# jluuser/PyTorch-VAE

Hardware: AMD Instinct MI355X
Metric: train images/sec @64x64x3 bs256 (curve tensors [B,64,6], SURVEY.md s0) (higher is better)
Workload: dtype f32; 1 GPU; C2: stage2_vq.yaml model with num_quantizers=1 K=512 D=64 N=64; full train step (fwd+loss+bwd+clip+AdamW+EMA), dropout 0.1, loss weights at epoch 100; per_gpu_batch=256, global_batch=256, seq_len=64, parallelism=dp1, hipgraph=True, params=43115078

## Files before the change

pytorch-vae_amd/csrc/loss.hip:

```cpp
#include "common.h"

namespace {

enum { T_VALID = 0, T_PAIR = 1, T_TRI = 2, T_QUAD = 3, T_FIVE = 4, T_ANY3 = 5, T_PDM = 8, T_LR = 40 };

enum {
    P_RAW = 0, P_ALN, P_BEST, P_RMSD_RAW, P_RMSD_BEST, P_CE, P_ACC, P_SSTV, P_BL, P_BA, P_DIR, P_DIH, P_TV2, P_TAU,
    P_PDM, P_LRPDM, P_WINK, P_COMMIT, P_KAPPA, P_COUNT
};

enum {
    M_LOSS = 0, M_REC_XYZ, M_MSE_RAW, M_MSE_ALN, M_REC_SS, M_SS_ACC, M_VQ_LOSS, M_BL, M_BA, M_DIR, M_DIH, M_GEOM,
    M_SS_TV, M_USAGE_REG, M_TV2, M_PPL, M_DEAD, M_RMSD_RAW, M_RMSD_ALN, M_PDM, M_WINK, M_KAPPA, M_TAU, M_LRPDM, M_COUNT
};

struct LossCfg {
    int B, L, Ntok, D;
    int Ls;
    const float* Ldev;
    int masked;
    int use_vq;
    float rmsd_w, ss_w, bl_w, ba_w, dir_w, dih_w, tv_l, pdm_w, wk_w, kap_w, tau_w, lr_w;
    float alpha, ss_tv_l, label_smoothing, beta;
    int pdm_window, wk_size, wk_stride, lr_sep, lr_stride, lr_max;
// ... 187 lines not shown
    }
    sm = block_sum_d(sm, dred);
    const double den = fmax(sm, 1.0);
    double amu[3], bmu[3];
    for (int c = 0; c < 3; ++c) { amu[c] = block_sum_d(sa[c], dred) / den; bmu[c] = block_sum_d(sb[c], dred) / den; }
    double Hm[9] = {0, 0, 0, 0, 0, 0, 0, 0, 0};
    for (int l = threadIdx.x; l < n; l += blockDim.x) {
        const double w = m[l0 + l];
        double ac[3], bc[3];
        for (int c = 0; c < 3; ++c) {
            ac[c] = (double)((float)a[3 * (l0 + l) + c] - (float)amu[c]);
            bc[c] = (double)((float)b[3 * (l0 + l) + c] - (float)bmu[c]);
        }
        for (int i = 0; i < 3; ++i)
            for (int j = 0; j < 3; ++j) Hm[3 * i + j] += w * ac[i] * bc[j];
    }
    for (int k = 0; k < 9; ++k) Hm[k] = block_sum_d(Hm[k], dred);
    if (threadIdx.x == 0) {
        double R[9];
        kabsch_rotation(Hm, R);
        bool ok = true;
        for (int k = 0; k < 9; ++k) { Rt_s[k] = (float)R[k]; ok = ok && isfinite(R[k]); }
        for (int j = 0; j < 3; ++j) {
            const double t = bmu[j] - (amu[0] * R[0 * 3 + j] + amu[1] * R[1 * 3 + j] + amu[2] * R[2 * 3 + j]);
            Rt_s[9 + j] = (float)t;
            ok = ok && isfinite(t);
        }
        Rt_s[12] = ok ? 1.f : 0.f;
    }
    __syncthreads();
    return Rt_s[12] != 0.f;
}

__global__ __launch_bounds__(256) void loss_counts_kernel(const unsigned char* __restrict__ mask, LossCfg c_in,
                                                          int* __restrict__ table) {
    const LossCfg c = loss_resolve(c_in);
    extern __shared__ unsigned char sm_[];
    unsigned char* m = sm_;
    const int b = blockIdx.x, L = c.L;
    for (int l = threadIdx.x; l < L; l += 256) m[l] = mask ? mask[(size_t)b * c.Ls + l] : 1;
    __syncthreads();
    int nv = 0, np = 0, nt = 0, nq = 0, n5 = 0;
    for (int l = threadIdx.x; l < L; l += 256) {
        nv += m[l];
        if (l + 1 < L) np += m[l] & m[l + 1];
        if (l + 2 < L) nt += m[l] & m[l + 1] & m[l + 2];
        if (l + 3 < L) nq += m[l] & m[l + 1] & m[l + 2] & m[l + 3];
        if (l + 4 < L) n5 += m[l] & m[l + 1] & m[l + 2] & m[l + 3] & m[l + 4];
    }
    __shared__ int red[5];
    if (threadIdx.x < 5) red[threadIdx.x] = 0;
    __syncthreads();
    atomicAdd(&red[0], nv); atomicAdd(&red[1], np); atomicAdd(&red[2], nt); atomicAdd(&red[3], nq); atomicAdd(&red[4], n5);
    __syncthreads();
    if (threadIdx.x == 0) {
        atomicAdd(&table[T_VALID], red[0]); atomicAdd(&table[T_PAIR], red[1]); atomicAdd(&table[T_TRI], red[2]);
        atomicAdd(&table[T_QUAD], red[3]); atomicAdd(&table[T_FIVE], red[4]);
        if (red[0] >= 3) atomicAdd(&table[T_ANY3], 1);
    }
    for (int d = 1 + (threadIdx.x >> 6); d < c.pdm_window && d < 32; d += 4) {
        int s = 0;
        for (int l = threadIdx.x & 63; l + d < L; l += 64) s += m[l] & m[l + d];
        for (int o = 32; o > 0; o >>= 1) s += __shfl_xor(s, o, 64);
        if ((threadIdx.x & 63) == 0 && s) atomicAdd(&table[T_PDM + d - 1], s);
    }
    {
        int p = 0;
        for (int off = 0; off < max(1, c.lr_max); ++off)
            for (int i = 0; i < L; i += max(1, c.lr_stride)) {
                const int j = i + c.lr_sep + off;
                if (j >= L) break;
                if ((p & 255) == (int)threadIdx.x && (m[i] & m[j])) atomicAdd(&table[T_LR + p], 1);
                ++p;
            }
    }
    for (int w = threadIdx.x; w < c.n_windows; w += 256) {
        const int s0 = w * max(1, c.wk_stride);
        int cnt = 0;
        for (int l = 0; l < c.wk_size; ++l) cnt += m[s0 + l];
        if (!c.masked || cnt >= 3) atomicAdd(&table[c.t_wk + w], 1);
    }
}

#define FOR_POS(n_) for (int base_ = 0; base_ < (n_); base_ += 256)

__global__ __launch_bounds__(256) void loss_sample_kernel(const float* __restrict__ recons,
                                                          const float* __restrict__ target,
                                                          const unsigned char* __restrict__ mask,
                                                          const float* __restrict__ ze, const float* __restrict__ zq,
                                                          const int* __restrict__ table, LossCfg c_in,
                                                          float* __restrict__ d_recons, float* __restrict__ d_ze,
                                                          float* __restrict__ part) {
    extern __shared__ __attribute__((aligned(16))) float sm[];
    const LossCfg c = loss_resolve(c_in);
    const int L = c.L, b = blockIdx.x, tid = threadIdx.x;
    double* dred = reinterpret_cast<double*>(sm);
    float* rx = sm + 8;
    float* gx = rx + 3 * L;
    float* lg = gx + 3 * L;
    float* pr = lg + 3 * L;
    float* g = pr + 3 * L;
    float* mk = g + 3 * L;
    float* dcs = mk + L;
    float* dhr = dcs + 2 * L;
    float* dhg = dhr + 2 * L;
    int* lab = reinterpret_cast<int*>(dhg + 2 * L);
    float* red = reinterpret_cast<float*>(lab + L);
    float* Rt = red + 4;
    float* rrb = Rt + 16;
    float* grb = rrb + 3 * L;
    float* gRb = grb + 3 * L;
    const float* rr = c.has_stats ? rrb : rx;
    const float* gr = c.has_stats ? grb : gx;
// ... 342 lines not shown
            }
        }
    }
    __syncthreads();

    float commit = 0.f;
    if (c.use_vq && ze) {
        const int n = c.Ntok * c.D;
        const float wq = 2.f * c.beta / ((float)c.B * (float)n);
        const float* zeb = ze + (size_t)b * n;
        const float* zqb = zq + (size_t)b * n;
        float* dzb = d_ze + (size_t)b * n;
        for (int i = tid; i < n; i += 256) {
            const float d = zeb[i] - zqb[i];
            commit += d * d;
            dzb[i] = wq * d;
        }
        commit = block_sum(commit, red);
    }

    float* dxb = d_recons + (size_t)b * c.Ls * 6;
    for (int l = tid; l < L; l += 256)
        for (int k = 0; k < 3; ++k) dxb[6 * l + k] = c.has_stats ? g[3 * l + k] + gRb[3 * l + k] * c.sd[k] : g[3 * l + k];
    for (int i = 6 * L + tid; i < 6 * c.Ls; i += 256) dxb[i] = 0.f;
    if (tid == 0) {
        float* p = part + (size_t)b * P_COUNT;
        p[P_RAW] = raw; p[P_ALN] = aln; p[P_BEST] = best;
        p[P_RMSD_RAW] = sqrtf(fmaxf(raw, 1e-12f)); p[P_RMSD_BEST] = sqrtf(fmaxf(best, 1e-12f));
        p[P_CE] = ce; p[P_ACC] = acc; p[P_SSTV] = sstv; p[P_BL] = bl; p[P_BA] = ba; p[P_DIR] = dr; p[P_DIH] = dih;
        p[P_TV2] = tv2; p[P_TAU] = tau; p[P_KAPPA] = kap; p[P_PDM] = pdm; p[P_LRPDM] = lrp; p[P_WINK] = wink; p[P_COMMIT] = commit;
    }
}

__global__ void loss_finish_kernel(const float* __restrict__ part, const int* __restrict__ table, LossCfg c_in,
                                   const float* __restrict__ vq_stats, float* __restrict__ metrics) {
    const LossCfg c = loss_resolve(c_in);
    __shared__ double acc[P_COUNT];
    if (threadIdx.x < P_COUNT) {
        double s = 0.0;
        for (int b = 0; b < c.B; ++b) s += (double)part[(size_t)b * P_COUNT + threadIdx.x];
        acc[threadIdx.x] = s;
    }
    __syncthreads();
    if (threadIdx.x != 0) return;
    auto cnt = [&](int slot) { return fmax((double)table[slot], 1.0); };
    const double B = c.B;
    const double l_raw = acc[P_RAW] / B, l_aln = acc[P_BEST] / B;
    const double l_xyz = c.alpha * l_aln + (1.0 - c.alpha) * l_raw;
    const double l_ss = acc[P_CE] / cnt(T_VALID);
    const double ss_tv = (c.ss_tv_l > 0.f && c.L >= 2) ? acc[P_SSTV] / cnt(T_PAIR) : 0.0;
    const double bl = c.L >= 2 ? acc[P_BL] / cnt(T_PAIR) : 0.0;
    const double ba = c.L >= 3 ? acc[P_BA] / cnt(T_TRI) : 0.0;
    const double dr = c.L >= 2 ? acc[P_DIR] / cnt(T_PAIR) : 0.0;
    double dih = 0.0;
    if (c.L >= 4) dih = c.masked ? acc[P_DIH] / cnt(T_QUAD) : acc[P_DIH] / (2.0 * B * (c.L - 3));
    const double geom = c.bl_w * bl + c.ba_w * ba + c.dir_w * dr + c.dih_w * dih;
    const double xyz_tv = (c.tv_l > 0.f && c.L >= 3) ? acc[P_TV2] / cnt(T_TRI) : 0.0;
    const double kappa = (c.kap_w > 0.f && c.L >= 3) ? acc[P_KAPPA] / cnt(T_TRI) : 0.0;
    const double tau = (c.tau_w > 0.f && c.L >= 5) ? acc[P_TAU] / cnt(T_FIVE) : 0.0;
    const double vq = c.use_vq ? c.beta * acc[P_COMMIT] / (B * c.Ntok * c.D) : 0.0;
    const double pdm = acc[P_PDM], lrp = acc[P_LRPDM], wink = acc[P_WINK];
    const double total = c.rmsd_w * l_xyz + c.ss_w * l_ss + vq + geom + c.ss_tv_l * ss_tv + c.tv_l * xyz_tv + c.pdm_w * pdm +
                         c.wk_w * wink + c.kap_w * kappa + c.tau_w * tau + c.lr_w * lrp;
    metrics[M_LOSS] = (float)total;
    metrics[M_REC_XYZ] = (float)l_xyz;
    metrics[M_MSE_RAW] = (float)l_raw;
    metrics[M_MSE_ALN] = (float)(acc[P_ALN] / B);
    metrics[M_REC_SS] = (float)l_ss;
    metrics[M_SS_ACC] = (float)(acc[P_ACC] / cnt(T_VALID));
    metrics[M_VQ_LOSS] = (float)vq;
    metrics[M_BL] = (float)bl; metrics[M_BA] = (float)ba; metrics[M_DIR] = (float)dr; metrics[M_DIH] = (float)dih;
    metrics[M_GEOM] = (float)geom;
    metrics[M_SS_TV] = (float)ss_tv;
    metrics[M_USAGE_REG] = 0.f;
    metrics[M_TV2] = (float)xyz_tv;
// ... 9 lines not shown

extern "C" int vqh_loss_fwd_bwd(const float* recons, const float* target, const unsigned char* mask, int masked,
                                const float* ze, const float* zq, const float* vq_stats, int B, int L, int L_stride, const float* L_dev,
                                int Ntok, int D, int use_vq, const float* weights, const int* iparams, const float* data_stats,
                                float* d_recons, float* d_ze, float* metrics, float* workspace,
                                long long workspace_floats, hipStream_t stream) {
    VQH_CHECK_ARG(B > 0 && L > 0 && L_stride >= L, "vqh_loss_fwd_bwd: bad shape");
    VQH_CHECK_ARG(recons && target && weights && iparams && d_recons && metrics && workspace, "vqh_loss_fwd_bwd: null pointer");
    VQH_CHECK_ARG(!use_vq || (ze && zq && d_ze), "vqh_loss_fwd_bwd: VQ tensors missing");
    LossCfg c{};
    c.B = B; c.L = L_dev ? L_stride : L; c.Ls = L_stride; c.Ldev = L_dev; c.Ntok = Ntok; c.D = D; c.masked = masked ? 1 : 0; c.use_vq = use_vq ? 1 : 0;
    c.rmsd_w = weights[0]; c.ss_w = weights[1]; c.bl_w = weights[2]; c.ba_w = weights[3]; c.dir_w = weights[4];
    c.dih_w = weights[5]; c.tv_l = weights[6]; c.pdm_w = weights[7]; c.wk_w = weights[8]; c.kap_w = weights[9];
    c.tau_w = weights[10]; c.lr_w = weights[11]; c.alpha = weights[12]; c.ss_tv_l = weights[13];
    c.label_smoothing = weights[14]; c.beta = weights[15];
    c.pdm_window = iparams[0]; c.wk_size = iparams[1]; c.wk_stride = iparams[2]; c.lr_sep = iparams[3];
    c.lr_stride = iparams[4]; c.lr_max = iparams[5];
    c.has_stats = data_stats ? 1 : 0;
    for (int k = 0; k < 3; ++k) { c.sd[k] = data_stats ? data_stats[k] : 1.f; c.mu[k] = data_stats ? data_stats[3 + k] : 0.f; }
    VQH_CHECK_ARG(c.pdm_window <= 33, "vqh_loss_fwd_bwd: pdm_window > 33 unsupported");
    int npairs = 0, nwin = 0;
    loss_enumerate(L_dev ? L_stride : L, c.lr_sep, c.lr_stride, c.lr_max, c.wk_size, c.wk_stride, &npairs, &nwin);
    c.n_lr_pairs = npairs;
    c.n_windows = nwin;
    c.t_wk = T_LR + npairs;
    const long long table_ints = c.t_wk + nwin + 8;
    const long long need = table_ints + (long long)B * P_COUNT;
    VQH_CHECK_ARG(need <= workspace_floats, "vqh_loss_fwd_bwd: workspace too small");
    int* table = reinterpret_cast<int*>(workspace);
    float* part = workspace + table_ints;
    hipError_t e = hipMemsetAsync(table, 0, sizeof(int) * table_ints, stream);
    if (e != hipSuccess) { vqh_set_error(hipGetErrorString(e)); return VQH_ERR_LAUNCH; }
    const int Lmax = c.L;
    hipLaunchKernelGGL(loss_counts_kernel, dim3(B), dim3(256), (size_t)Lmax, stream, mask, c, table);
    const size_t smem = sizeof(float) * (size_t)(8 + 23 * Lmax + 4 + 16 + 9 * Lmax + 4);
    VQH_CHECK_ARG(smem <= 160 * 1024, "vqh_loss_fwd_bwd: sequence too long for the LDS-resident loss kernel");
    static bool attr_set = false;
    if (!attr_set) {
        hipError_t ea = hipFuncSetAttribute(reinterpret_cast<const void*>(&loss_sample_kernel),
                                            hipFuncAttributeMaxDynamicSharedMemorySize, 160 * 1024);
        if (ea != hipSuccess) { vqh_set_error(hipGetErrorString(ea)); return VQH_ERR_LAUNCH; }
        attr_set = true;
    }
    hipLaunchKernelGGL(loss_sample_kernel, dim3(B), dim3(256), smem, stream, recons, target, mask, ze, zq, table, c,
                       d_recons, d_ze, part);
    hipLaunchKernelGGL(loss_finish_kernel, dim3(1), dim3(64), 0, stream, part, table, c, vq_stats, metrics);
    VQH_LAUNCH_CHECK();
    return VQH_OK;
}
```

pytorch-vae_amd/csrc/rowwise.hip:

```cpp
#include "common.h"
#include <stdlib.h>

namespace {

constexpr int WAVES_PER_BLOCK = 4;

__global__ __launch_bounds__(256) void layernorm_fwd_kernel(const float* __restrict__ x, int ldx,
                                                            const float* __restrict__ w, const float* __restrict__ b,
                                                            float* __restrict__ y, int ldy, float* __restrict__ mean,
                                                            float* __restrict__ rstd, int rows, int H, float eps) {
    const int lane = threadIdx.x & 63;
    const int row = blockIdx.x * WAVES_PER_BLOCK + (threadIdx.x >> 6);
    if (row >= rows) return;
    const float* xr = x + (size_t)row * ldx;
    float s = 0.f;
    for (int i = lane; i < H; i += 64) s += xr[i];
    const float mu = wave_sum(s) / (float)H;
    float v = 0.f;
    for (int i = lane; i < H; i += 64) {
        const float d = xr[i] - mu;
        v += d * d;
    }
    const float rs = rsqrtf(wave_sum(v) / (float)H + eps);
    float* yr = y + (size_t)row * ldy;
    for (int i = lane; i < H; i += 64) yr[i] = (xr[i] - mu) * rs * w[i] + b[i];
    if (lane == 0) {
        if (mean) mean[row] = mu;
        if (rstd) rstd[row] = rs;
    }
}

template <int NV>
__global__ __launch_bounds__(256) void layernorm_fwd_vec_kernel(const float* __restrict__ x, int ldx,
                                                                const float* __restrict__ w, const float* __restrict__ b,
                                                                float* __restrict__ y, int ldy, float* __restrict__ mean,
                                                                float* __restrict__ rstd, int rows, int H, float eps) {
    const int lane = threadIdx.x & 63, wave = threadIdx.x >> 6;
    const int nq = H >> 2;
// ... 209 lines not shown
        for (int j = 0; j < 16; ++j) t += red[j][tx];
        float* o = (i < H) ? dw + i : db + (i - H);
        *o = (beta != 0.f) ? beta * (*o) + t : t;
    }
}

__global__ __launch_bounds__(1024) void reduce_slabs_kernel(const float* __restrict__ slabs, int S, long long stride,
                                                            long long n, float* __restrict__ out, float beta) {
    __shared__ float red[16][64];
    const int tx = threadIdx.x & 63, ty = threadIdx.x >> 6;
    const long long i = (long long)blockIdx.x * 64 + tx;
    float s = 0.f;
    if (i < n) {
        int k = ty;
        for (; k + 48 < S; k += 64) {
            const float a = slabs[(size_t)k * stride + i], b = slabs[(size_t)(k + 16) * stride + i];
            const float c = slabs[(size_t)(k + 32) * stride + i], d = slabs[(size_t)(k + 48) * stride + i];
            s += (a + b) + (c + d);
        }
        for (; k < S; k += 16) s += slabs[(size_t)k * stride + i];
    }
    red[ty][tx] = s;
    __syncthreads();
    if (ty == 0 && i < n) {
        float t = 0.f;
#pragma unroll
        for (int j = 0; j < 16; ++j) t += red[j][tx];
        out[i] = (beta != 0.f) ? beta * out[i] + t : t;
    }
}

__global__ __launch_bounds__(256) void colsum_vec_kernel(const float* __restrict__ X, int ld, int M, int N,
                                                         float* __restrict__ part, int rows_per_block) {
    __shared__ f32x4 red[4][64];
    const int lane = threadIdx.x & 63, ry = threadIdx.x >> 6;
    const int c = blockIdx.x * 256 + lane * 4;
    const int r0 = blockIdx.y * rows_per_block;
    const int r1 = min(M, r0 + rows_per_block);
    f32x4 s0 = {0.f, 0.f, 0.f, 0.f}, s1 = s0;
    if (c < N) {
        int r = r0 + ry;
        for (; r + 4 < r1; r += 8) {
            s0 += *reinterpret_cast<const f32x4*>(X + (size_t)r * ld + c);
            s1 += *reinterpret_cast<const f32x4*>(X + (size_t)(r + 4) * ld + c);
        }
        for (; r < r1; r += 4) s0 += *reinterpret_cast<const f32x4*>(X + (size_t)r * ld + c);
    }
    red[ry][lane] = s0 + s1;
    __syncthreads();
    if (ry == 0 && c < N) {
        const f32x4 t = (red[0][lane] + red[1][lane]) + (red[2][lane] + red[3][lane]);
        *reinterpret_cast<f32x4*>(part + (size_t)blockIdx.y * N + c) = t;
    }
}

__global__ __launch_bounds__(256) void colsum_kernel(const float* __restrict__ X, int ld, int M, int N,
                                                     float* __restrict__ part, int rows_per_block) {
    __shared__ float red[4][64];
    const int c = blockIdx.x * 64 + (threadIdx.x & 63);
    const int ry = threadIdx.x >> 6;
    const int r0 = blockIdx.y * rows_per_block;
    const int r1 = min(M, r0 + rows_per_block);
    float s = 0.f;
    if (c < N)
        for (int r = r0 + ry; r < r1; r += 4) s += X[(size_t)r * ld + c];
    red[ry][threadIdx.x & 63] = s;
    __syncthreads();
    if (ry == 0 && c < N)
        part[(size_t)blockIdx.y * N + c] = red[0][threadIdx.x] + red[1][threadIdx.x] + red[2][threadIdx.x] + red[3][threadIdx.x];
}

__global__ __launch_bounds__(256) void embed_fwd_kernel(const float* __restrict__ x, int ldx, int c0,
                                                        const float* __restrict__ W, const float* __restrict__ b,
                                                        const float* __restrict__ pe, float* __restrict__ out,
                                                        int rows, int L, int H, DropCfg drop) {
    unsigned dkey = 0;
    if (drop.p > 0.f) dkey = drop_key(drop, drop.rng_state[0], drop.rng_state[1]);
    const long long total = (long long)rows * H;
    for (long long e = (long long)blockIdx.x * blockDim.x + threadIdx.x; e < total; e += (long long)gridDim.x * blockDim.x) {
        const int r = (int)(e / H), hcol = (int)(e % H);
        const float* xr = x + (size_t)r * ldx + c0;
        float v = b[hcol] + W[hcol * 3 + 0] * xr[0] + W[hcol * 3 + 1] * xr[1] + W[hcol * 3 + 2] * xr[2];
        if (drop.p > 0.f) v *= drop_keep(drop, dkey, (unsigned long long)e);
        out[e] = v + pe[(size_t)(r % L) * H + hcol];
    }
}

__global__ __launch_bounds__(256) void embed_bwd_kernel(const float* __restrict__ dy, const float* __restrict__ x,
                                                        int ldx, int c0, float* __restrict__ part, int rows, int H,
                                                        int rows_per_block, DropCfg drop) {
    __shared__ float red[4][4][64];
    unsigned dkey = 0;
    if (drop.p > 0.f) dkey = drop_key(drop, drop.rng_state[0], drop.rng_state[1]);
    const int hcol = blockIdx.x * 64 + (threadIdx.x & 63);
    const int ry = threadIdx.x >> 6;
    const int r0 = blockIdx.y * rows_per_block, r1 = min(rows, r0 + rows_per_block);
    float a0 = 0.f, a1 = 0.f, a2 = 0.f, a3 = 0.f;
    if (hcol < H)
        for (int r = r0 + ry; r < r1; r += 4) {
            float d = dy[(size_t)r * H + hcol];
            if (drop.p > 0.f) d *= drop_keep(drop, dkey, (unsigned long long)r * H + hcol);
            const float* xr = x + (size_t)r * ldx + c0;
            a0 += d * xr[0];
            a1 += d * xr[1];
            a2 += d * xr[2];
            a3 += d;
        }
    const int l = threadIdx.x & 63;
    red[ry][0][l] = a0; red[ry][1][l] = a1; red[ry][2][l] = a2; red[ry][3][l] = a3;
    __syncthreads();
    if (ry == 0 && hcol < H) {
#pragma unroll
        for (int c = 0; c < 4; ++c)
            part[((size_t)blockIdx.y * 4 + c) * H + hcol] = red[0][c][l] + red[1][c][l] + red[2][c][l] + red[3][c][l];
    }
}

__global__ void bcast_rows_kernel(const float* __restrict__ p0, const float* __restrict__ p1, float* __restrict__ out,
                                  int B, long long n) {
    const long long total = (long long)B * n;
    for (long long e = (long long)blockIdx.x * blockDim.x + threadIdx.x; e < total; e += (long long)gridDim.x * blockDim.x) {
        const long long i = e % n;
        out[e] = p1 ? p0[i] + p1[i] : p0[i];
    }
}

__global__ void dropout_bwd_kernel(const float* __restrict__ dy, float* __restrict__ out, long long n, DropCfg drop) {
    const unsigned dkey = drop_key(drop, drop.rng_state[0], drop.rng_state[1]);
    const long long nq = (n + 3) / 4;
    for (long long q = (long long)blockIdx.x * blockDim.x + threadIdx.x; q < nq; q += (long long)gridDim.x * blockDim.x) {
        float f[4];
        drop4(drop, dkey, (unsigned long long)q, f);
#pragma unroll
        for (int e = 0; e < 4; ++e) {
            const long long i = q * 4 + e;
            if (i < n) out[i] = dy[i] * f[e];
        }
    }
}

__global__ void add_kernel(const float* __restrict__ a, const float* __restrict__ b, float* __restrict__ out, long long n) {
    for (long long i = (long long)blockIdx.x * blockDim.x + threadIdx.x; i < n; i += (long long)gridDim.x * blockDim.x)
        out[i] = a[i] + b[i];
}

__global__ void sigmoid_bwd_kernel(const float* __restrict__ dy, const float* __restrict__ y, float* __restrict__ out, long long n) {
    for (long long i = (long long)blockIdx.x * blockDim.x + threadIdx.x; i < n; i += (long long)gridDim.x * blockDim.x)
        out[i] = dy[i] * y[i] * (1.f - y[i]);
}

__global__ void copy2d_kernel(const float* __restrict__ src, int lds_, float* __restrict__ dst, int ldd, int rows, int cols) {
    const long long total = (long long)rows * cols;
    for (long long e = (long long)blockIdx.x * blockDim.x + threadIdx.x; e < total; e += (long long)gridDim.x * blockDim.x) {
        const int r = (int)(e / cols), c = (int)(e % cols);
        dst[(size_t)r * ldd + c] = src[(size_t)r * lds_ + c];
    }
// ... 172 lines not shown
#define LN_BWD(V)                                                                                                  \
    hipLaunchKernelGGL((layernorm_bwd_kernel<V>), dim3(nblk), dim3(256), 0, stream, dy, lddy, x, ldx, w, mean, rstd, \
                       dx, lddx, accumulate_dx, workspace, rows, H)
    if (H <= 64) LN_BWD(1);
    else if (H <= 128) LN_BWD(2);
    else if (H <= 256) LN_BWD(4);
    else if (H <= 512) LN_BWD(8);
    else if (H <= 1024) LN_BWD(16);
    else LN_BWD(32);
#undef LN_BWD
#undef LN_BWD_V
    VQH_LAUNCH_CHECK();
    if (dx_drop && !vec) {
        VQH_CHECK_ARG(lddx == H, "vqh_layernorm_bwd: dx_drop on the unaligned path needs a dense dx");
        hipLaunchKernelGGL(dropout_bwd_kernel, dim3(blocks_for(((long long)rows * H + 3) / 4)), dim3(256), 0, stream, dx, dx_drop,
                           (long long)rows * H, dcfg);
    }
    hipLaunchKernelGGL(reduce_slabs2_kernel, dim3((2 * H + 63) / 64), dim3(1024), 0, stream, workspace, nblk, H, dw, db, beta);
    VQH_LAUNCH_CHECK();
    return VQH_OK;
}

extern "C" int vqh_colsum(const float* X, int ld, int M, int N, float* out, float beta, float* workspace,
                          long long workspace_floats, hipStream_t stream) {
    VQH_CHECK_ARG(M >= 0 && N >= 0 && ld >= N, "vqh_colsum: bad shape");
    if (N == 0) return VQH_OK;
    VQH_CHECK_ARG(out && workspace, "vqh_colsum: null pointer");
    int rb = (M + 255) / 256;
    if (rb < 1) rb = 1;
    if (rb > 128) rb = 128;
    const int rows_per_block = (M + rb - 1) / rb > 0 ? (M + rb - 1) / rb : 1;
    VQH_CHECK_ARG((long long)rb * N <= workspace_floats, "vqh_colsum: workspace too small");
    if ((N & 3) == 0 && (ld & 3) == 0 && (reinterpret_cast<uintptr_t>(X) & 15) == 0 && (reinterpret_cast<uintptr_t>(workspace) & 15) == 0)
        hipLaunchKernelGGL(colsum_vec_kernel, dim3((N + 255) / 256, rb), dim3(256), 0, stream, X, ld, M, N, workspace, rows_per_block);
    else
        hipLaunchKernelGGL(colsum_kernel, dim3((N + 63) / 64, rb), dim3(256), 0, stream, X, ld, M, N, workspace, rows_per_block);
    hipLaunchKernelGGL(reduce_slabs_kernel, dim3((N + 63) / 64), dim3(1024), 0, stream, workspace, rb, (long long)N,
                       (long long)N, out, beta);
    VQH_LAUNCH_CHECK();
    return VQH_OK;
}

extern "C" int vqh_embed_fwd(const float* x, int ldx, int col0, const float* W, const float* b, const float* pe,
                             float* out, int rows, int L, int H, const unsigned long long* rng_state,
                             unsigned drop_site, float drop_p, hipStream_t stream) {
    VQH_CHECK_ARG(rows >= 0 && L > 0 && H > 0 && ldx >= col0 + 3, "vqh_embed_fwd: bad shape");
    if (rows == 0) return VQH_OK;
    VQH_CHECK_ARG(x && W && b && pe && out, "vqh_embed_fwd: null pointer");
    VQH_CHECK_ARG(drop_p == 0.f || rng_state, "vqh_embed_fwd: dropout needs rng_state");
    DropCfg d = make_drop(rng_state, drop_site, drop_p);
    hipLaunchKernelGGL(embed_fwd_kernel, dim3(blocks_for((long long)rows * H)), dim3(256), 0, stream, x, ldx, col0, W, b,
                       pe, out, rows, L, H, d);
    VQH_LAUNCH_CHECK();
    return VQH_OK;
}

extern "C" int vqh_embed_bwd(const float* dy, const float* x, int ldx, int col0, float* dW, float* db, float beta,
                             int rows, int H, const unsigned long long* rng_state, unsigned drop_site, float drop_p,
                             float* workspace, long long workspace_floats, hipStream_t stream) {
    VQH_CHECK_ARG(rows >= 0 && H > 0, "vqh_embed_bwd: bad shape");
    VQH_CHECK_ARG(dy && x && dW && db && workspace, "vqh_embed_bwd: null pointer");
    VQH_CHECK_ARG(drop_p == 0.f || rng_state, "vqh_embed_bwd: dropout needs rng_state");
    int rb = (rows + 255) / 256;
    if (rb < 1) rb = 1;
    if (rb > 128) rb = 128;
    const int rpb = (rows + rb - 1) / rb > 0 ? (rows + rb - 1) / rb : 1;
    VQH_CHECK_ARG((long long)rb * 4 * H <= workspace_floats, "vqh_embed_bwd: workspace too small");
    DropCfg d = make_drop(rng_state, drop_site, drop_p);
    hipLaunchKernelGGL(embed_bwd_kernel, dim3((H + 63) / 64, rb), dim3(256), 0, stream, dy, x, ldx, col0, workspace, rows,
                       H, rpb, d);
    VQH_LAUNCH_CHECK();
    float* scratch = workspace + (size_t)rb * 4 * H;
    VQH_CHECK_ARG((long long)rb * 4 * H + 4 * H <= workspace_floats, "vqh_embed_bwd: workspace too small");
    hipLaunchKernelGGL(reduce_slabs_kernel, dim3((4 * H + 63) / 64), dim3(1024), 0, stream, workspace, rb,
                       (long long)4 * H, (long long)4 * H, scratch, 0.f);
    hipLaunchKernelGGL(embed_scatter_kernel, dim3((H + 255) / 256), dim3(256), 0, stream, scratch, dW, db, beta, H);
    VQH_LAUNCH_CHECK();
    return VQH_OK;
}

extern "C" int vqh_bcast_rows(const float* p0, const float* p1, float* out, int B, long long n, hipStream_t stream) {
    VQH_CHECK_ARG(B >= 0 && n >= 0, "vqh_bcast_rows: bad shape");
    if (B == 0 || n == 0) return VQH_OK;
    hipLaunchKernelGGL(bcast_rows_kernel, dim3(blocks_for((long long)B * n)), dim3(256), 0, stream, p0, p1, out, B, n);
    VQH_LAUNCH_CHECK();
    return VQH_OK;
}

extern "C" int vqh_dropout_bwd(const float* dy, float* out, long long n, const unsigned long long* rng_state,
                               unsigned drop_site, float drop_p, hipStream_t stream) {
    VQH_CHECK_ARG(n >= 0 && drop_p > 0.f && drop_p < 1.f && rng_state, "vqh_dropout_bwd: bad argument");
    if (n == 0) return VQH_OK;
    DropCfg d = make_drop(rng_state, drop_site, drop_p);
    hipLaunchKernelGGL(dropout_bwd_kernel, dim3(blocks_for((n + 3) / 4)), dim3(256), 0, stream, dy, out, n, d);
    VQH_LAUNCH_CHECK();
    return VQH_OK;
}

extern "C" int vqh_add(const float* a, const float* b, float* out, long long n, hipStream_t stream) {
    VQH_CHECK_ARG(n >= 0, "vqh_add: bad n");
    if (n == 0) return VQH_OK;
    hipLaunchKernelGGL(add_kernel, dim3(blocks_for(n)), dim3(256), 0, stream, a, b, out, n);
    VQH_LAUNCH_CHECK();
    return VQH_OK;
}

extern "C" int vqh_copy2d(const float* src, int lds_, float* dst, int ldd, int rows, int cols, hipStream_t stream) {
    VQH_CHECK_ARG(rows >= 0 && cols >= 0 && lds_ >= cols && ldd >= cols, "vqh_copy2d: bad shape");
    if (rows == 0 || cols == 0) return VQH_OK;
    hipLaunchKernelGGL(copy2d_kernel, dim3(blocks_for((long long)rows * cols)), dim3(256), 0, stream, src, lds_, dst, ldd,
                       rows, cols);
    VQH_LAUNCH_CHECK();
    return VQH_OK;
}

extern "C" int vqh_sigmoid_bwd(const float* dy, const float* y, float* out, long long n, hipStream_t stream) {
    VQH_CHECK_ARG(n >= 0, "vqh_sigmoid_bwd: bad n");
    if (n == 0) return VQH_OK;
    hipLaunchKernelGGL(sigmoid_bwd_kernel, dim3(blocks_for(n)), dim3(256), 0, stream, dy, y, out, n);
    VQH_LAUNCH_CHECK();
    return VQH_OK;
}

extern "C" int vqh_memset(void* ptr, int value, long long bytes, hipStream_t stream) {
    VQH_CHECK_ARG(bytes >= 0, "vqh_memset: bad size");
    if (bytes == 0) return VQH_OK;
    hipError_t e = hipMemsetAsync(ptr, value, (size_t)bytes, stream);
// ... 47 lines not shown
```

Baseline: 9933 images/s.

## Vectorize embed, broadcast, dropout and colsum kernels; bit-pack loss mask counts

Replaces the per-sample mask-count kernel with a multi-sample kernel that packs the mask into 64-bit ballot words, counts with popcount and accumulates into an LDS table before the global atomics. Adds float4-vectorized variants for embedding forward and backward, row broadcast and dropout backward, and widens the colsum kernel's row unrolling. The loss finish kernel now stages partials through LDS using 256 threads. The goal is fewer scalar memory transactions and fewer global atomics in small elementwise and reduction kernels, at the cost of more code paths with alignment and shape gates. Explicit non-contracted multiply and add calls are used to keep rounding identical to the scalar paths.

```diff
diff --git a/pytorch-vae_amd/csrc/loss.hip b/pytorch-vae_amd/csrc/loss.hip
--- a/pytorch-vae_amd/csrc/loss.hip
+++ b/pytorch-vae_amd/csrc/loss.hip
@@ -243,53 +243,90 @@
     return Rt_s[12] != 0.f;
 }
 
+constexpr int COUNT_BLOCKS = 64;
+constexpr int COUNT_WORDS = 32;
+constexpr int COUNT_LDS_INTS = 8 * 1024;
+
 __global__ __launch_bounds__(256) void loss_counts_kernel(const unsigned char* __restrict__ mask, LossCfg c_in,
-                                                          int* __restrict__ table) {
+                                                          int* __restrict__ table, int table_ints, int lds_table, int spb) {
+    typedef unsigned long long u64;
     const LossCfg c = loss_resolve(c_in);
-    extern __shared__ unsigned char sm_[];
-    unsigned char* m = sm_;
-    const int b = blockIdx.x, L = c.L;
-    for (int l = threadIdx.x; l < L; l += 256) m[l] = mask ? mask[(size_t)b * c.Ls + l] : 1;
-    __syncthreads();
-    int nv = 0, np = 0, nt = 0, nq = 0, n5 = 0;
-    for (int l = threadIdx.x; l < L; l += 256) {
-        nv += m[l];
-        if (l + 1 < L) np += m[l] & m[l + 1];
-        if (l + 2 < L) nt += m[l] & m[l + 1] & m[l + 2];
-        if (l + 3 < L) nq += m[l] & m[l + 1] & m[l + 2] & m[l + 3];
-        if (l + 4 < L) n5 += m[l] & m[l + 1] & m[l + 2] & m[l + 3] & m[l + 4];
-    }
-    __shared__ int red[5];
-    if (threadIdx.x < 5) red[threadIdx.x] = 0;
-    __syncthreads();
-    atomicAdd(&red[0], nv); atomicAdd(&red[1], np); atomicAdd(&red[2], nt); atomicAdd(&red[3], nq); atomicAdd(&red[4], n5);
-    __syncthreads();
-    if (threadIdx.x == 0) {
-        atomicAdd(&table[T_VALID], red[0]); atomicAdd(&table[T_PAIR], red[1]); atomicAdd(&table[T_TRI], red[2]);
-        atomicAdd(&table[T_QUAD], red[3]); atomicAdd(&table[T_FIVE], red[4]);
-        if (red[0] >= 3) atomicAdd(&table[T_ANY3], 1);
-    }
-    for (int d = 1 + (threadIdx.x >> 6); d < c.pdm_window && d < 32; d += 4) {
-        int s = 0;
-        for (int l = threadIdx.x & 63; l + d < L; l += 64) s += m[l] & m[l + d];
-        for (int o = 32; o > 0; o >>= 1) s += __shfl_xor(s, o, 64);
-        if ((threadIdx.x & 63) == 0 && s) atomicAdd(&table[T_PDM + d - 1], s);
-    }
-    {
-        int p = 0;
-        for (int off = 0; off < max(1, c.lr_max); ++off)
-            for (int i = 0; i < L; i += max(1, c.lr_stride)) {
-                const int j = i + c.lr_sep + off;
-                if (j >= L) break;
-                if ((p & 255) == (int)threadIdx.x && (m[i] & m[j])) atomicAdd(&table[T_LR + p], 1);
-                ++p;
-            }
-    }
-    for (int w = threadIdx.x; w < c.n_windows; w += 256) {
-        const int s0 = w * max(1, c.wk_stride);
-        int cnt = 0;
-        for (int l = 0; l < c.wk_size; ++l) cnt += m[s0 + l];
-        if (!c.masked || cnt >= 3) atomicAdd(&table[c.t_wk + w], 1);
+    extern __shared__ __attribute__((aligned(16))) unsigned char sm_[];
+    const int lane = threadIdx.x & 63, wave = threadIdx.x >> 6, L = c.L;
+    const int nw = (L + 63) >> 6, pitch = ((c.Ls + 63) >> 6) + 1;
+    u64* words = reinterpret_cast<u64*>(sm_);
+    int* tab = lds_table ? reinterpret_cast<int*>(sm_ + (size_t)spb * pitch * sizeof(u64)) : table;
+    const int b0 = blockIdx.x * spb, nb = min(spb, c.B - b0);
+    if (lds_table)
+        for (int i = threadIdx.x; i < table_ints; i += 256) tab[i] = 0;
+    const int nitems = nb * nw;
+    constexpr int U = 8;
+    for (int i0 = wave * U; i0 < nitems; i0 += 4 * U) {
+        bool v[U];
+#pragma unroll
+        for (int u = 0; u < U; ++u) {
+            const int item = i0 + u, s = item / nw, l = 64 * (item - s * nw) + lane;
+            v[u] = item < nitems && l < L && (mask ? mask[(size_t)(b0 + s) * c.Ls + l] != 0 : true);
+        }
+#pragma unroll
+        for (int u = 0; u < U; ++u) {
+            const int item = i0 + u, s = item / nw;
+            const u64 word = __ballot(v[u]);
+            if (lane == 0 && item < nitems) words[s * pitch + (item - s * nw)] = word;
+        }
+    }
+    for (int s = threadIdx.x; s < nb; s += 256) words[s * pitch + nw] = 0ull;
+    __syncthreads();
+    const int st_lr = max(1, c.lr_stride), st_wk = max(1, c.wk_stride), n_off = max(1, c.lr_max);
+    for (int s = wave; s < nb; s += 4) {
+        const u64* mw = words + s * pitch;
+        auto bit = [&](int l) { return (int)((mw[l >> 6] >> (l & 63)) & 1ull); };
+        auto shifted = [&](int w, int d) { return d ? (mw[w] >> d) | (mw[w + 1] << (64 - d)) : mw[w]; };
+        if (lane < 5) {
+            int n = 0;
+            for (int w = 0; w < nw; ++w) {
+                u64 a = mw[w];
+                for (int k = 1; k <= lane; ++k) a &= shifted(w, k);
+                n += __popcll(a);
+            }
+            if (n) atomicAdd(&tab[T_VALID + lane], n);
+            if (lane == 0 && n >= 3) atomicAdd(&tab[T_ANY3], 1);
+        } else if (lane >= 8 && lane < 8 + 31) {
+            const int d = lane - 7;
+            if (d < c.pdm_window) {
+                int n = 0;
+                for (int w = 0; w < nw; ++w) n += __popcll(mw[w] & shifted(w, d));
+                if (n) atomicAdd(&tab[T_PDM + d - 1], n);
+            }
+        }
+        for (int p = lane; p < c.n_lr_pairs; p += 64) {
+            int off = 0, k = p;
+            for (; off < n_off; ++off) {
+                const int room = L - c.lr_sep - off;
+                const int cntp = room > 0 ? (room + st_lr - 1) / st_lr : 0;
+                if (k < cntp) break;
+                k -= cntp;
+            }
+            const int i = k * st_lr, j = i + c.lr_sep + off;
+            if (off < n_off && (bit(i) & bit(j))) atomicAdd(&tab[T_LR + p], 1);
+        }
+        for (int w = lane; w < c.n_windows; w += 64) {
+            const int s0 = w * st_wk;
+            int cnt = 0;
+            for (int o = 0; o < c.wk_size; o += 64) {
+                u64 x = shifted((s0 + o) >> 6, (s0 + o) & 63);
+                if (c.wk_size - o < 64) x &= (1ull << (c.wk_size - o)) - 1ull;
+                cnt += __popcll(x);
+            }
+            if (!c.masked || cnt >= 3) atomicAdd(&tab[c.t_wk + w], 1);
+        }
+    }
+    if (lds_table) {
+        __syncthreads();
+        for (int i = threadIdx.x; i < table_ints; i += 256) {
+            const int v = tab[i];
+            if (v) atomicAdd(&table[i], v);
+        }
     }
 }
 
@@ -698,15 +735,24 @@
     }
 }
 
-__global__ void loss_finish_kernel(const float* __restrict__ part, const int* __restrict__ table, LossCfg c_in,
-                                   const float* __restrict__ vq_stats, float* __restrict__ metrics) {
+constexpr int FINISH_THREADS = 256, FINISH_CHUNK = 256;
+
+__global__ __launch_bounds__(FINISH_THREADS) void loss_finish_kernel(const float* __restrict__ part, const int* __restrict__ table,
+                                                                     LossCfg c_in, const float* __restrict__ vq_stats,
+                                                                     float* __restrict__ metrics) {
     const LossCfg c = loss_resolve(c_in);
     __shared__ double acc[P_COUNT];
-    if (threadIdx.x < P_COUNT) {
-        double s = 0.0;
-        for (int b = 0; b < c.B; ++b) s += (double)part[(size_t)b * P_COUNT + threadIdx.x];
-        acc[threadIdx.x] = s;
-    }
+    __shared__ float stage[FINISH_CHUNK * P_COUNT];
+    double s = 0.0;
+    for (int b0 = 0; b0 < c.B; b0 += FINISH_CHUNK) {
+        const int nb = min(FINISH_CHUNK, c.B - b0);
+        __syncthreads();
+        for (int i = threadIdx.x; i < nb * P_COUNT; i += FINISH_THREADS) stage[i] = part[(size_t)b0 * P_COUNT + i];
+        __syncthreads();
+        if (threadIdx.x < P_COUNT)
+            for (int b = 0; b < nb; ++b) s += (double)stage[b * P_COUNT + threadIdx.x];
+    }
+    if (threadIdx.x < P_COUNT) acc[threadIdx.x] = s;
     __syncthreads();
     if (threadIdx.x != 0) return;
     auto cnt = [&](int slot) { return fmax((double)table[slot], 1.0); };
@@ -782,7 +828,21 @@
     hipError_t e = hipMemsetAsync(table, 0, sizeof(int) * table_ints, stream);
     if (e != hipSuccess) { vqh_set_error(hipGetErrorString(e)); return VQH_ERR_LAUNCH; }
     const int Lmax = c.L;
-    hipLaunchKernelGGL(loss_counts_kernel, dim3(B), dim3(256), (size_t)Lmax, stream, mask, c, table);
+    {
+        const int lds_table = table_ints <= COUNT_LDS_INTS ? 1 : 0;
+        const size_t tab_bytes = lds_table ? sizeof(int) * (size_t)table_ints : 0;
+        const long long pitch = (L_stride + 63) / 64 + 1;
+        long long nblk = ((long long)B * (pitch - 1) + COUNT_WORDS - 1) / COUNT_WORDS;
+        if (nblk > COUNT_BLOCKS) nblk = COUNT_BLOCKS;
+        long long spb = (B + nblk - 1) / nblk;
+        const long long spb_fit = (long long)((32 * 1024) / (pitch * sizeof(unsigned long long)));
+        VQH_CHECK_ARG(spb_fit >= 1, "vqh_loss_fwd_bwd: sequence too long for the count kernel");
+        if (spb > spb_fit) spb = spb_fit;
+        nblk = (B + spb - 1) / spb;
+        const size_t csmem = (size_t)spb * pitch * sizeof(unsigned long long) + tab_bytes;
+        hipLaunchKernelGGL(loss_counts_kernel, dim3((unsigned)nblk), dim3(256), csmem, stream, mask, c, table, (int)table_ints,
+                           lds_table, (int)spb);
+    }
     const size_t smem = sizeof(float) * (size_t)(8 + 23 * Lmax + 4 + 16 + 9 * Lmax + 4);
     VQH_CHECK_ARG(smem <= 160 * 1024, "vqh_loss_fwd_bwd: sequence too long for the LDS-resident loss kernel");
     static bool attr_set = false;
@@ -794,7 +854,7 @@
     }
     hipLaunchKernelGGL(loss_sample_kernel, dim3(B), dim3(256), smem, stream, recons, target, mask, ze, zq, table, c,
                        d_recons, d_ze, part);
-    hipLaunchKernelGGL(loss_finish_kernel, dim3(1), dim3(64), 0, stream, part, table, c, vq_stats, metrics);
+    hipLaunchKernelGGL(loss_finish_kernel, dim3(1), dim3(FINISH_THREADS), 0, stream, part, table, c, vq_stats, metrics);
     VQH_LAUNCH_CHECK();
     return VQH_OK;
 }
diff --git a/pytorch-vae_amd/csrc/rowwise.hip b/pytorch-vae_amd/csrc/rowwise.hip
--- a/pytorch-vae_amd/csrc/rowwise.hip
+++ b/pytorch-vae_amd/csrc/rowwise.hip
@@ -4,6 +4,15 @@
 namespace {
 
 constexpr int WAVES_PER_BLOCK = 4;
+
+__device__ __forceinline__ float mul_sep(float a, float b) {
+#pragma clang fp contract(off)
+    return a * b;
+}
+__device__ __forceinline__ float add_sep(float a, float b) {
+#pragma clang fp contract(off)
+    return a + b;
+}
 
 __global__ __launch_bounds__(256) void layernorm_fwd_kernel(const float* __restrict__ x, int ldx,
                                                             const float* __restrict__ w, const float* __restrict__ b,
@@ -279,24 +288,28 @@
 
 __global__ __launch_bounds__(256) void colsum_vec_kernel(const float* __restrict__ X, int ld, int M, int N,
                                                          float* __restrict__ part, int rows_per_block) {
-    __shared__ f32x4 red[4][64];
-    const int lane = threadIdx.x & 63, ry = threadIdx.x >> 6;
-    const int c = blockIdx.x * 256 + lane * 4;
+    __shared__ f32x4 red[8][32];
+    const int cl = threadIdx.x & 31, rl = threadIdx.x >> 5;
+    const int c = blockIdx.x * 128 + cl * 4;
     const int r0 = blockIdx.y * rows_per_block;
     const int r1 = min(M, r0 + rows_per_block);
-    f32x4 s0 = {0.f, 0.f, 0.f, 0.f}, s1 = s0;
+    f32x4 s = {0.f, 0.f, 0.f, 0.f};
     if (c < N) {
-        int r = r0 + ry;
-        for (; r + 4 < r1; r += 8) {
-            s0 += *reinterpret_cast<const f32x4*>(X + (size_t)r * ld + c);
-            s1 += *reinterpret_cast<const f32x4*>(X + (size_t)(r + 4) * ld + c);
-        }
-        for (; r < r1; r += 4) s0 += *reinterpret_cast<const f32x4*>(X + (size_t)r * ld + c);
-    }
-    red[ry][lane] = s0 + s1;
+        const float* Xc = X + c;
+        int r = r0 + rl;
+        for (; r + 56 < r1; r += 64) {
+            f32x4 v[8];
+#pragma unroll
+            for (int u = 0; u < 8; ++u) v[u] = *reinterpret_cast<const f32x4*>(Xc + (size_t)(r + 8 * u) * ld);
+#pragma unroll
+            for (int u = 0; u < 8; ++u) s += v[u];
+        }
+        for (; r < r1; r += 8) s += *reinterpret_cast<const f32x4*>(Xc + (size_t)r * ld);
+    }
+    red[rl][cl] = s;
     __syncthreads();
-    if (ry == 0 && c < N) {
-        const f32x4 t = (red[0][lane] + red[1][lane]) + (red[2][lane] + red[3][lane]);
+    if (rl == 0 && c < N) {
+        const f32x4 t = ((red[0][cl] + red[4][cl]) + (red[1][cl] + red[5][cl])) + ((red[2][cl] + red[6][cl]) + (red[3][cl] + red[7][cl]));
         *reinterpret_cast<f32x4*>(part + (size_t)blockIdx.y * N + c) = t;
     }
 }
@@ -333,6 +346,115 @@
     }
 }
 
+constexpr long long EMBED_VEC_MIN_ELEMS = 1 << 20;
+template <int NV>
+__global__ __launch_bounds__(256) void embed_fwd_vec_kernel(const float* __restrict__ x, int ldx, int c0,
+                                                            const float* __restrict__ W, const float* __restrict__ b,
+                                                            const float* __restrict__ pe, float* __restrict__ out,
+                                                            int rows, int L, int H, DropCfg drop) {
+    unsigned dkey = 0;
+    if (drop.p > 0.f) dkey = drop_key(drop, drop.rng_state[0], drop.rng_state[1]);
+    const int lane = threadIdx.x & 63, wave = threadIdx.x >> 6;
+    const int nq = H >> 2;
+    f32x4 w0[NV], w1[NV], w2[NV], bv[NV];
+#pragma unroll
+    for (int j = 0; j < NV; ++j) {
+        const int q = lane + 64 * j;
+        const f32x4 z = {0.f, 0.f, 0.f, 0.f};
+        w0[j] = (q < nq) ? *reinterpret_cast<const f32x4*>(W + 12 * q) : z;
+        w1[j] = (q < nq) ? *reinterpret_cast<const f32x4*>(W + 12 * q + 4) : z;
+        w2[j] = (q < nq) ? *reinterpret_cast<const f32x4*>(W + 12 * q + 8) : z;
+        bv[j] = (q < nq) ? *reinterpret_cast<const f32x4*>(b + 4 * q) : z;
+    }
+    for (int r = blockIdx.x * WAVES_PER_BLOCK + wave; r < rows; r += gridDim.x * WAVES_PER_BLOCK) {
+        const float* xr = x + (size_t)r * ldx + c0;
+        const float x0 = xr[0], x1 = xr[1], x2 = xr[2];
+        const float* per = pe + (size_t)(r % L) * H;
+        float* outr = out + (size_t)r * H;
+#pragma unroll
+        for (int j = 0; j < NV; ++j) {
+            const int q = lane + 64 * j;
+            if (q < nq) {
+                f32x4 v;
+                v[0] = fmaf(w0[j][2], x2, fmaf(w0[j][1], x1, fmaf(w0[j][0], x0, bv[j][0])));
+                v[1] = fmaf(w1[j][1], x2, fmaf(w1[j][0], x1, fmaf(w0[j][3], x0, bv[j][1])));
+                v[2] = fmaf(w2[j][0], x2, fmaf(w1[j][3], x1, fmaf(w1[j][2], x0, bv[j][2])));
+                v[3] = fmaf(w2[j][3], x2, fmaf(w2[j][2], x1, fmaf(w2[j][1], x0, bv[j][3])));
+                if (drop.p > 0.f) {
+                    float f[4];
+                    drop4(drop, dkey, (unsigned long long)r * nq + q, f);
+#pragma unroll
+                    for (int e = 0; e < 4; ++e) v[e] = mul_sep(v[e], f[e]);
+                }
+                const f32x4 pv = *reinterpret_cast<const f32x4*>(per + 4 * q);
+#pragma unroll
+                for (int e = 0; e < 4; ++e) v[e] = add_sep(v[e], pv[e]);
+                *reinterpret_cast<f32x4*>(outr + 4 * q) = v;
+            }
+        }
+    }
+}
+
+__global__ __launch_bounds__(128) void embed_bwd_vec_kernel(const float* __restrict__ dy, const float* __restrict__ x,
+                                                            int ldx, int c0, float* __restrict__ part, int rows, int H,
+                                                            int rows_per_block, DropCfg drop) {
+    __shared__ f32x4 red[4][4][32];
+    unsigned dkey = 0;
+    if (drop.p > 0.f) dkey = drop_key(drop, drop.rng_state[0], drop.rng_state[1]);
+    const int cl = threadIdx.x & 31, ry = threadIdx.x >> 5;
+    const int hcol = blockIdx.x * 128 + cl * 4;
+    const int nq = H >> 2;
+    const int r0 = blockIdx.y * rows_per_block, r1 = min(rows, r0 + rows_per_block);
+    const f32x4 z = {0.f, 0.f, 0.f, 0.f};
+    f32x4 a0 = z, a1 = z, a2 = z, a3 = z;
+    if (hcol < H) {
+        constexpr int U = 8;
+        for (int rb = r0 + ry; rb < r1; rb += 4 * U) {
+            f32x4 d[U];
+            float xs[U][3];
+#pragma unroll
+            for (int u = 0; u < U; ++u) {
+                const int r = rb + 4 * u;
+                d[u] = z;
+                xs[u][0] = xs[u][1] = xs[u][2] = 0.f;
+                if (r < r1) {
+                    d[u] = *reinterpret_cast<const f32x4*>(dy + (size_t)r * H + hcol);
+                    const float* xr = x + (size_t)r * ldx + c0;
+                    xs[u][0] = xr[0]; xs[u][1] = xr[1]; xs[u][2] = xr[2];
+                }
+            }
+#pragma unroll
+            for (int u = 0; u < U; ++u) {
+                const int r = rb + 4 * u;
+                if (r < r1) {
+                    f32x4 dd = d[u];
+                    if (drop.p > 0.f) {
+                        float f[4];
+                        drop4(drop, dkey, (unsigned long long)r * nq + (hcol >> 2), f);
+#pragma unroll
+                        for (int e = 0; e < 4; ++e) dd[e] = mul_sep(dd[e], f[e]);
+                    }
+#pragma unroll
+                    for (int e = 0; e < 4; ++e) {
+                        a0[e] = add_sep(a0[e], mul_sep(dd[e], xs[u][0]));
+                        a1[e] = fmaf(dd[e], xs[u][1], a1[e]);
+                        a2[e] = fmaf(dd[e], xs[u][2], a2[e]);
+                        a3[e] = add_sep(a3[e], dd[e]);
+                    }
+                }
+            }
+        }
+    }
+    red[ry][0][cl] = a0; red[ry][1][cl] = a1; red[ry][2][cl] = a2; red[ry][3][cl] = a3;
+    __syncthreads();
+    if (ry == 0 && hcol < H) {
+#pragma unroll
+        for (int c = 0; c < 4; ++c)
+            *reinterpret_cast<f32x4*>(part + ((size_t)blockIdx.y * 4 + c) * H + hcol) =
+                red[0][c][cl] + red[1][c][cl] + red[2][c][cl] + red[3][c][cl];
+    }
+}
+
 __global__ __launch_bounds__(256) void embed_bwd_kernel(const float* __restrict__ dy, const float* __restrict__ x,
                                                         int ldx, int c0, float* __restrict__ part, int rows, int H,
                                                         int rows_per_block, DropCfg drop) {
@@ -346,12 +468,12 @@
     if (hcol < H)
         for (int r = r0 + ry; r < r1; r += 4) {
             float d = dy[(size_t)r * H + hcol];
-            if (drop.p > 0.f) d *= drop_keep(drop, dkey, (unsigned long long)r * H + hcol);
+            if (drop.p > 0.f) d = mul_sep(d, drop_keep(drop, dkey, (unsigned long long)r * H + hcol));
             const float* xr = x + (size_t)r * ldx + c0;
-            a0 += d * xr[0];
-            a1 += d * xr[1];
-            a2 += d * xr[2];
-            a3 += d;
+            a0 = add_sep(a0, mul_sep(d, xr[0]));
+            a1 = fmaf(d, xr[1], a1);
+            a2 = fmaf(d, xr[2], a2);
+            a3 = add_sep(a3, d);
         }
     const int l = threadIdx.x & 63;
     red[ry][0][l] = a0; red[ry][1][l] = a1; red[ry][2][l] = a2; red[ry][3][l] = a3;
@@ -369,6 +491,28 @@
     for (long long e = (long long)blockIdx.x * blockDim.x + threadIdx.x; e < total; e += (long long)gridDim.x * blockDim.x) {
         const long long i = e % n;
         out[e] = p1 ? p0[i] + p1[i] : p0[i];
+    }
+}
+
+__global__ __launch_bounds__(256) void bcast_rows_vec_kernel(const float* __restrict__ p0, const float* __restrict__ p1,
+                                                             float* __restrict__ out, int B, long long n) {
+    const long long nq = n >> 2;
+    for (long long q = (long long)blockIdx.x * blockDim.x + threadIdx.x; q < nq; q += (long long)gridDim.x * blockDim.x) {
+        f32x4 v = *reinterpret_cast<const f32x4*>(p0 + 4 * q);
+        if (p1) v = v + *reinterpret_cast<const f32x4*>(p1 + 4 * q);
+        for (int b = blockIdx.y; b < B; b += gridDim.y) *reinterpret_cast<f32x4*>(out + (size_t)b * n + 4 * q) = v;
+    }
+}
+
+__global__ __launch_bounds__(256) void dropout_bwd_vec_kernel(const float* __restrict__ dy, float* __restrict__ out,
+                                                              long long nq, DropCfg drop) {
+    const unsigned dkey = drop_key(drop, drop.rng_state[0], drop.rng_state[1]);
+    for (long long q = (long long)blockIdx.x * blockDim.x + threadIdx.x; q < nq; q += (long long)gridDim.x * blockDim.x) {
+        float f[4];
+        drop4(drop, dkey, (unsigned long long)q, f);
+        f32x4 v = *reinterpret_cast<const f32x4*>(dy + 4 * q);
+        v[0] *= f[0]; v[1] *= f[1]; v[2] *= f[2]; v[3] *= f[3];
+        *reinterpret_cast<f32x4*>(out + 4 * q) = v;
     }
 }
 
@@ -607,7 +751,7 @@
     const int rows_per_block = (M + rb - 1) / rb > 0 ? (M + rb - 1) / rb : 1;
     VQH_CHECK_ARG((long long)rb * N <= workspace_floats, "vqh_colsum: workspace too small");
     if ((N & 3) == 0 && (ld & 3) == 0 && (reinterpret_cast<uintptr_t>(X) & 15) == 0 && (reinterpret_cast<uintptr_t>(workspace) & 15) == 0)
-        hipLaunchKernelGGL(colsum_vec_kernel, dim3((N + 255) / 256, rb), dim3(256), 0, stream, X, ld, M, N, workspace, rows_per_block);
+        hipLaunchKernelGGL(colsum_vec_kernel, dim3((N + 127) / 128, rb), dim3(256), 0, stream, X, ld, M, N, workspace, rows_per_block);
     else
         hipLaunchKernelGGL(colsum_kernel, dim3((N + 63) / 64, rb), dim3(256), 0, stream, X, ld, M, N, workspace, rows_per_block);
     hipLaunchKernelGGL(reduce_slabs_kernel, dim3((N + 63) / 64), dim3(1024), 0, stream, workspace, rb, (long long)N,
@@ -624,8 +768,22 @@
     VQH_CHECK_ARG(x && W && b && pe && out, "vqh_embed_fwd: null pointer");
     VQH_CHECK_ARG(drop_p == 0.f || rng_state, "vqh_embed_fwd: dropout needs rng_state");
     DropCfg d = make_drop(rng_state, drop_site, drop_p);
-    hipLaunchKernelGGL(embed_fwd_kernel, dim3(blocks_for((long long)rows * H)), dim3(256), 0, stream, x, ldx, col0, W, b,
-                       pe, out, rows, L, H, d);
+    const bool vec = (H % 4 == 0) && H <= 1024 && (long long)rows * H >= EMBED_VEC_MIN_ELEMS &&
+                     (((reinterpret_cast<uintptr_t>(W) | reinterpret_cast<uintptr_t>(b) | reinterpret_cast<uintptr_t>(pe) |
+                        reinterpret_cast<uintptr_t>(out)) & 15) == 0);
+    if (vec) {
+        int gv = (rows + WAVES_PER_BLOCK - 1) / WAVES_PER_BLOCK;
+        if (gv > 2048) gv = 2048;
+#define EMBED_FWD_V(V)                                                                                                  \
+    hipLaunchKernelGGL((embed_fwd_vec_kernel<V>), dim3(gv), dim3(256), 0, stream, x, ldx, col0, W, b, pe, out, rows, L, H, d)
+        if (H <= 256) EMBED_FWD_V(1);
+        else if (H <= 512) EMBED_FWD_V(2);
+        else EMBED_FWD_V(4);
+#undef EMBED_FWD_V
+    } else {
+        hipLaunchKernelGGL(embed_fwd_kernel, dim3(blocks_for((long long)rows * H)), dim3(256), 0, stream, x, ldx, col0, W, b,
+                           pe, out, rows, L, H, d);
+    }
     VQH_LAUNCH_CHECK();
     return VQH_OK;
 }
@@ -642,8 +800,12 @@
     const int rpb = (rows + rb - 1) / rb > 0 ? (rows + rb - 1) / rb : 1;
     VQH_CHECK_ARG((long long)rb * 4 * H <= workspace_floats, "vqh_embed_bwd: workspace too small");
     DropCfg d = make_drop(rng_state, drop_site, drop_p);
-    hipLaunchKernelGGL(embed_bwd_kernel, dim3((H + 63) / 64, rb), dim3(256), 0, stream, dy, x, ldx, col0, workspace, rows,
-                       H, rpb, d);
+    if ((H & 3) == 0 && ((reinterpret_cast<uintptr_t>(dy) | reinterpret_cast<uintptr_t>(workspace)) & 15) == 0)
+        hipLaunchKernelGGL(embed_bwd_vec_kernel, dim3((H + 127) / 128, rb), dim3(128), 0, stream, dy, x, ldx, col0, workspace,
+                           rows, H, rpb, d);
+    else
+        hipLaunchKernelGGL(embed_bwd_kernel, dim3((H + 63) / 64, rb), dim3(256), 0, stream, dy, x, ldx, col0, workspace, rows,
+                           H, rpb, d);
     VQH_LAUNCH_CHECK();
     float* scratch = workspace + (size_t)rb * 4 * H;
     VQH_CHECK_ARG((long long)rb * 4 * H + 4 * H <= workspace_floats, "vqh_embed_bwd: workspace too small");
@@ -657,7 +819,14 @@
 extern "C" int vqh_bcast_rows(const float* p0, const float* p1, float* out, int B, long long n, hipStream_t stream) {
     VQH_CHECK_ARG(B >= 0 && n >= 0, "vqh_bcast_rows: bad shape");
     if (B == 0 || n == 0) return VQH_OK;
-    hipLaunchKernelGGL(bcast_rows_kernel, dim3(blocks_for((long long)B * n)), dim3(256), 0, stream, p0, p1, out, B, n);
+    if ((n & 3) == 0 && ((reinterpret_cast<uintptr_t>(p0) | reinterpret_cast<uintptr_t>(p1) | reinterpret_cast<uintptr_t>(out)) & 15) == 0) {
+        const int gx = blocks_for(n >> 2, 256, 1024);
+        int gy = (2048 + gx - 1) / gx;
+        if (gy > B) gy = B;
+        hipLaunchKernelGGL(bcast_rows_vec_kernel, dim3(gx, gy), dim3(256), 0, stream, p0, p1, out, B, n);
+    } else {
+        hipLaunchKernelGGL(bcast_rows_kernel, dim3(blocks_for((long long)B * n)), dim3(256), 0, stream, p0, p1, out, B, n);
+    }
     VQH_LAUNCH_CHECK();
     return VQH_OK;
 }
@@ -667,7 +836,10 @@
     VQH_CHECK_ARG(n >= 0 && drop_p > 0.f && drop_p < 1.f && rng_state, "vqh_dropout_bwd: bad argument");
     if (n == 0) return VQH_OK;
     DropCfg d = make_drop(rng_state, drop_site, drop_p);
-    hipLaunchKernelGGL(dropout_bwd_kernel, dim3(blocks_for((n + 3) / 4)), dim3(256), 0, stream, dy, out, n, d);
+    if ((n & 3) == 0 && ((reinterpret_cast<uintptr_t>(dy) | reinterpret_cast<uintptr_t>(out)) & 15) == 0)
+        hipLaunchKernelGGL(dropout_bwd_vec_kernel, dim3(blocks_for(n >> 2)), dim3(256), 0, stream, dy, out, n >> 2, d);
+    else
+        hipLaunchKernelGGL(dropout_bwd_kernel, dim3(blocks_for((n + 3) / 4)), dim3(256), 0, stream, dy, out, n, d);
     VQH_LAUNCH_CHECK();
     return VQH_OK;
 }
```

After: 10010 images/s, median of 6. Within noise of the previous version (+0.8%).
